# Linketic/TC-Light

Measured on AMD Instinct MI355X. Metric: relit frames/sec end-to-end (denoise+2-stage opt), higher is better.
Workload: dtype f16

## Files before the change

tc_light_amd/csrc/attn.hip:

```cpp
#include "common.h"
#include "gemm_conv.h"
#include "prof.h"
#include "../../include/tclight_hip.h"
#include <stdlib.h>
#include <type_traits>

typedef _Float16 half8 __attribute__((ext_vector_type(8)));
typedef _Float16 half4 __attribute__((ext_vector_type(4)));
typedef float float16v __attribute__((ext_vector_type(16)));
typedef float float4v __attribute__((ext_vector_type(4)));
typedef unsigned u32x4 __attribute__((ext_vector_type(4)));
typedef unsigned u32x2 __attribute__((ext_vector_type(2)));

#ifndef TCL_FLASH80_DEFAULT
#define TCL_FLASH80_DEFAULT 4
#endif
#ifndef TCL_FLASH_PV32_DEFAULT
#define TCL_FLASH_PV32_DEFAULT 0
#endif
#define KV_TILE 64
#define V_STRIDE 72
#ifndef TCL_DPV40
#define TCL_DPV40 64
#endif
// ... 36 lines not shown
        for (int j = 0; j < 8; ++j) tile[r * st + c8 + j] = x[j];
    }
    __syncthreads();
    _Float16* out = vt + ((long)bh * ntiles + tile_idx) * vt_tile_halves(DPV);
    for (int i = threadIdx.x; i < DPV * 64; i += 256) {
        int dd = i / 64, r = i % 64;
        _Float16 val = tile[r * st + dd];
        if (dd == d && DPV > d) val = (t0 + r < T) ? (_Float16)1.f : (_Float16)0.f;
        int pr = (r & ~12) | ((r & 4) << 1) | ((r & 8) >> 1);
        if (skew && (((dd & 15) + 4) & 8)) pr ^= 16;
        out[dd * V_STRIDE + pr] = val;
    }
}
__global__ __launch_bounds__(256) void k_pack_vt(const _Float16* __restrict__ v, long bstride, int ld, int T, int H, int d,
                                                 _Float16* __restrict__ vt, int ntiles, int DPV, int skew) {
    pack_vt_blk(blockIdx.x, blockIdx.y, v, bstride, ld, T, H, d, vt, ntiles, DPV, skew);
}
struct PackRows { const _Float16* src; long bstride; int ld, T, d; float scale; _Float16* dst; int Tp, DP; long total; int one_col; };
__global__ __launch_bounds__(256) void k_pack_qkv(PackRows q, PackRows k, int gq, int gk, int H, const _Float16* __restrict__ v, long vbs, int ldv, int Tk, int d,
                                                  _Float16* __restrict__ vt, int ntiles, int DPV, int skew) {
    const int blk = blockIdx.x;
    if (blk < gq) pack_rows_blk(blk, gq, q.src, q.bstride, q.ld, q.T, H, q.d, q.scale, q.dst, q.Tp, q.DP, q.total, q.one_col);
    else if (blk < gq + gk) pack_rows_blk(blk - gq, gk, k.src, k.bstride, k.ld, k.T, H, k.d, k.scale, k.dst, k.Tp, k.DP, k.total, k.one_col);
    else { const int i = blk - gq - gk; pack_vt_blk(i % ntiles, i / ntiles, v, vbs, ldv, Tk, H, d, vt, ntiles, DPV, skew); }
}

__device__ __attribute__((aligned(1024))) unsigned g_flash_zero[256];

__device__ __forceinline__ float xhalf_max(float v) {
    const auto r = __builtin_amdgcn_permlane32_swap(__float_as_uint(v), __float_as_uint(v), false, false);
    return fmaxf(__uint_as_float(r[0]), __uint_as_float(r[1]));
}

template <int D, int DP, int DPV, int QB, int NSTG, int TPB, int MINB, int SPEC, int PVW, int NW, bool SPLIT = false>
__device__ __forceinline__ void flash_block(const int bid, const _Float16* __restrict__ Qp, const _Float16* __restrict__ Kp, const _Float16* __restrict__ Vt,
                                            _Float16* __restrict__ O, int H, int Tq, int Tk, int Tqp, int Tkp, int d, int ldo, long obstride,
                                            int kv_div, int nqb, int* __restrict__ flags, float* __restrict__ lse = nullptr) {
    constexpr int KS = DP + 8;
    constexpr int NQK = DP / 16, NDT = DPV / 32;
    constexpr int KBYTES = KV_TILE * KS * 2, VBYTES = vt_tile_halves(DPV) * 2, SBYTES = KBYTES + VBYTES;
    constexpr int NPIECE = (SBYTES + 1023) / 1024, NPW = (NPIECE + NW - 1) / NW, SSTRIDE = NPIECE * 1024;
    constexpr bool LROW = DPV > D;
    constexpr bool FOLD = DP > D && LROW && (D % 16 == 8);
    constexpr bool PVQ = QB > 1;
    constexpr bool PV16 = PVW == 16 && D == 40 && LROW && DPV >= 48;
    constexpr int NT16 = 3;
    extern __shared__ __attribute__((aligned(16))) char smem[];

    const int head = bid % H, qb_ = (bid / H) % nqb, b = bid / (H * nqb);
    const int tid = threadIdx.x, lane = tid & 63, wid = __builtin_amdgcn_readfirstlane(tid >> 6), hl = lane >> 5, ql = lane & 31;
    const int q0 = qb_ * (32 * NW * QB) + wid * (32 * QB);
    const long bh = (long)b * H + head, kbh = (long)(b / kv_div) * H + head;
    const int nt = Tkp / KV_TILE, nfull = Tk / KV_TILE;
    const char* kbase = (const char*)(Kp + kbh * Tkp * KS);
    const char* vbase = (const char*)(Vt + kbh * nt * vt_tile_halves(DPV));
    const char* zero = (const char*)g_flash_zero;

#ifdef TCL_FLASH_PRIO_EXP
    if ((bid >> 3) & 1) __builtin_amdgcn_s_setprio(TCL_FLASH_PRIO_EXP);
#endif
    half8 qf[QB][NQK];
#pragma unroll
    for (int qb = 0; qb < QB; ++qb) {
        const _Float16* qrow = Qp + (bh * Tqp + q0 + qb * 32 + ql) * DP + 8 * hl;
#pragma unroll
        for (int ks = 0; ks < NQK; ++ks) qf[qb][ks] = *(const half8*)(qrow + ks * 16);
    }
    static_assert(KBYTES % 1024 == 0, "K image must be piece-aligned");
    const int lane16 = lane * 16;
    __attribute__((address_space(3))) char* const lds0 = (__attribute__((address_space(3))) char*)smem;
#define FLASH_ISSUE(IT)                                                                                                       \
    {                                                                                                                         \
        const char* kt_ = kbase + (long)(IT) * KBYTES;                                                                        \
        const char* vt_ = vbase + (long)(IT) * VBYTES;                                                                        \
        const int st_ = ((IT) % NSTG) * SSTRIDE;                                                                              \
        _Pragma("unroll") for (int i = 0; i < NPW; ++i) {                                                                    \
            const int pb_ = (wid + NW * i) * 1024;                                                                            \
            const char* src_ = (pb_ < KBYTES ? kt_ + pb_ : vt_ + (pb_ - KBYTES)) + lane16;                                    \
            if (SBYTES % 1024 != 0) src_ = pb_ + lane16 < SBYTES ? src_ : zero + lane16;                                      \
            else if (NSTG != 3 && NPW * NW != NPIECE && (wid + NW * i) >= NPIECE) continue;    \
            const int dst_ = (wid + NW * i) < NPIECE ? st_ + pb_ : NSTG * SSTRIDE;        \
            __builtin_amdgcn_global_load_lds((const __attribute__((address_space(1))) void*)src_,                             \
                                             (__attribute__((address_space(3))) void*)(lds0 + dst_), 16, 0, 0);               \
        }                                                                                                                     \
    }

    float16v o[QB][PV16 ? 1 : NDT];
    float4v o16[QB][2][PV16 ? NT16 : 1];
    float m[QB], lsum[QB];
#pragma unroll
    for (int qb = 0; qb < QB; ++qb) {
        m[qb] = FOLD ? 0.f : -1e30f; lsum[qb] = 0.f;
#pragma unroll
        for (int t = 0; t < (PV16 ? 1 : NDT); ++t)
#pragma unroll
            for (int r = 0; r < 16; ++r) o[qb][t][r] = 0.f;
#pragma unroll
        for (int qt = 0; qt < 2; ++qt)
#pragma unroll
            for (int t = 0; t < (PV16 ? NT16 : 1); ++t) o16[qb][qt][t] = float4v{0.f, 0.f, 0.f, 0.f};
    }

#ifndef TCL_SPEC_OFF
#define TCL_SPEC_OFF 3
#endif
    constexpr float OFF = TCL_SPEC_OFF;
    unsigned orv = 0;
    static_assert(!SPEC || (FOLD && (PV16 || PVQ)), "the speculative softmax is the head_dim-40 path");
    auto rebase = [&](const int it, const bool first) __attribute__((always_inline)) {
        if constexpr (SPEC) {
        const _Float16* kt = (const _Float16*)(smem + (it % NSTG) * SSTRIDE);
#pragma unroll
        for (int qb = 0; qb < QB; ++qb) {
            float16v s[2];
#pragma unroll
            for (int blk = 0; blk < 2; ++blk) {
#pragma unroll
                for (int r = 0; r < 16; ++r) s[blk][r] = 0.f;
#pragma unroll
                for (int ks = 0; ks < NQK; ++ks)
                    s[blk] = __builtin_amdgcn_mfma_f32_32x32x16_f16(*(const half8*)(kt + (blk * 32 + ql) * KS + 8 * hl + ks * 16), qf[qb][ks], s[blk], 0, 0, 0);
            }
            float mx = -1e30f;
#pragma unroll
            for (int blk = 0; blk < 2; ++blk)
#pragma unroll
                for (int r = 0; r < 16; ++r) mx = fmaxf(mx, s[blk][r]);
            mx = xhalf_max(mx) + OFF;
            const float mn = (float)(_Float16)(m[qb] + (first ? mx : fmaxf(mx, 0.f)));
            const float delta = mn - m[qb], alpha = __builtin_amdgcn_exp2f(-delta);
            m[qb] = mn;
            if (hl == 1) qf[qb][D / 16][0] = (_Float16)(-mn);
            if (!first) {
                if constexpr (PV16) {
#pragma unroll
                    for (int qt = 0; qt < 2; ++qt) {
                        const float aq = __shfl(alpha, (lane & 15) + 16 * qt, 64);
#pragma unroll
                        for (int t = 0; t < NT16; ++t) o16[qb][qt][t] *= aq;
                    }
                } else {
#pragma unroll
                    for (int t = 0; t < NDT; ++t)
#pragma unroll
                        for (int r = 0; r < 16; ++r) o[qb][t][r] *= alpha;
                }
            }
        }
        }
    };
    auto tile = [&](const int it, auto MK) __attribute__((always_inline)) {
        const _Float16* kt = (const _Float16*)(smem + (it % NSTG) * SSTRIDE);
        const _Float16* vt = kt + KV_TILE * KS;
        constexpr bool mask = decltype(MK)::value;
        half8 kf[2][NQK];
#pragma unroll
        for (int blk = 0; blk < 2; ++blk)
#pragma unroll
            for (int ks = 0; ks < NQK; ++ks) kf[blk][ks] = *(const half8*)(kt + (blk * 32 + ql) * KS + 8 * hl + ks * 16);
        half8 pf[QB][2][2];
        half8 vfr[PVQ && !PV16 ? 2 : 1][2][NDT];
        half8 vf16[PV16 ? 2 : 1][NT16];
        if constexpr (PV16) {
            const int goff = (((lane >> 4) & 1) * 16 + (lane >> 5) * 8) ^ ((((lane & 15) + 4) & 8) ? 16 : 0);
#pragma unroll
            for (int blk = 0; blk < 2; ++blk)
#pragma unroll
                for (int t = 0; t < NT16; ++t) vf16[blk][t] = *(const half8*)(vt + (t * 16 + (lane & 15)) * V_STRIDE + blk * 32 + goff);
        } else if constexpr (PVQ) {
#pragma unroll
            for (int blk = 0; blk < 2; ++blk)
#pragma unroll
                for (int ss = 0; ss < 2; ++ss)
#pragma unroll
                    for (int t = 0; t < NDT; ++t) vfr[blk][ss][t] = *(const half8*)(vt + (ql + t * 32) * V_STRIDE + blk * 32 + 16 * ss + 8 * hl);
        }
        float16v sacc[QB][2];
#pragma unroll
        for (int qb = 0; qb < QB; ++qb)
#pragma unroll
            for (int blk = 0; blk < 2; ++blk) {
#pragma unroll
                for (int r = 0; r < 16; ++r) sacc[qb][blk][r] = 0.f;
#pragma unroll
                for (int ks = 0; ks < NQK; ++ks) sacc[qb][blk] = __builtin_amdgcn_mfma_f32_32x32x16_f16(kf[blk][ks], qf[qb][ks], sacc[qb][blk], 0, 0, 0);
// ... 25 lines not shown
                        const half8 p0 = __builtin_bit_cast(half8, x), p1 = __builtin_bit_cast(half8, y);
#pragma unroll
                        for (int t = 0; t < NT16; ++t) {
                            o16[qb][0][t] = __builtin_amdgcn_mfma_f32_16x16x32_f16(vf16[blk][t], p0, o16[qb][0][t], 0, 0, 0);
                            o16[qb][1][t] = __builtin_amdgcn_mfma_f32_16x16x32_f16(vf16[blk][t], p1, o16[qb][1][t], 0, 0, 0);
                        }
                    } else {
#pragma unroll
                        for (int ss = 0; ss < 2; ++ss)
#pragma unroll
                            for (int t = 0; t < NDT; ++t) o[qb][t] = __builtin_amdgcn_mfma_f32_32x32x16_f16(vfr[blk][ss][t], pf[qb][blk][ss], o[qb][t], 0, 0, 0);
                    }
                }
            }
            if constexpr (TPB == 1) {
                if (__any((orv & 0x40004000u) != 0u)) {
                    asm volatile("; rebase");
                    rebase(it, false);
                }
                orv = 0;
            }
            return;
        }
        float mxq[QB];
#pragma unroll
        for (int qb = 0; qb < QB; ++qb) {
            float mx = sacc[qb][0][0];
#pragma unroll
            for (int blk = 0; blk < 2; ++blk)
#pragma unroll
                for (int r = 0; r < 16; ++r) mx = fmaxf(mx, sacc[qb][blk][r]);
            mxq[qb] = xhalf_max(mx);
        }
        bool need = it == 0;
#pragma unroll
        for (int qb = 0; qb < QB; ++qb) need |= FOLD ? (mxq[qb] > 6.f) : (mxq[qb] > m[qb] + 6.f);
        if (__any(need)) {
            asm volatile("; rebase");
#pragma unroll
            for (int qb = 0; qb < QB; ++qb) {
                float16v (&s)[2] = sacc[qb];
                const float mx = mxq[qb];
                if constexpr (FOLD) {
                    if (it == 0 || __any(mx > 6.f)) {
                        const float mn = (float)(_Float16)(m[qb] + (it == 0 ? mx : fmaxf(mx, 0.f)));
                        const float delta = mn - m[qb], alpha = __builtin_amdgcn_exp2f(-delta);
                        m[qb] = mn;
                        if (hl == 1) qf[qb][D / 16][0] = (_Float16)(-mn);
                        if constexpr (PV16) {
#pragma unroll
                            for (int qt = 0; qt < 2; ++qt) {
                                const float aq = __shfl(alpha, (lane & 15) + 16 * qt, 64);
#pragma unroll
                                for (int t = 0; t < NT16; ++t) o16[qb][qt][t] *= aq;
                            }
                        } else {
#pragma unroll
                            for (int t = 0; t < NDT; ++t)
#pragma unroll
                                for (int r = 0; r < 16; ++r) o[qb][t][r] *= alpha;
                        }
#pragma unroll
                        for (int blk = 0; blk < 2; ++blk)
#pragma unroll
                            for (int r = 0; r < 16; ++r) s[blk][r] -= delta;
                    }
                } else if (__any(mx > m[qb] + 6.f)) {
                    const float mn = fmaxf(m[qb], mx), alpha = __builtin_amdgcn_exp2f(m[qb] - mn);
                    m[qb] = mn;
                    lsum[qb] *= alpha;
#pragma unroll
                    for (int t = 0; t < NDT; ++t)
#pragma unroll
                        for (int r = 0; r < 16; ++r) o[qb][t][r] *= alpha;
                }
            }
        }
#pragma unroll
// ... 24 lines not shown
                    const half8 p0 = __builtin_bit_cast(half8, x), p1 = __builtin_bit_cast(half8, y);
#pragma unroll
                    for (int t = 0; t < NT16; ++t) {
                        o16[qb][0][t] = __builtin_amdgcn_mfma_f32_16x16x32_f16(vf16[blk][t], p0, o16[qb][0][t], 0, 0, 0);
                        o16[qb][1][t] = __builtin_amdgcn_mfma_f32_16x16x32_f16(vf16[blk][t], p1, o16[qb][1][t], 0, 0, 0);
                    }
                }
            } else if constexpr (PVQ) {
#pragma unroll
                for (int blk = 0; blk < 2; ++blk)
#pragma unroll
                    for (int ss = 0; ss < 2; ++ss)
#pragma unroll
                        for (int t = 0; t < NDT; ++t) o[qb][t] = __builtin_amdgcn_mfma_f32_32x32x16_f16(vfr[blk][ss][t], pf[qb][blk][ss], o[qb][t], 0, 0, 0);
            }
        }
        if constexpr (!PVQ && !PV16) {
#pragma unroll
            for (int blk = 0; blk < 2; ++blk)
#pragma unroll
                for (int ss = 0; ss < 2; ++ss) {
                    const _Float16* vr = vt + ql * V_STRIDE + blk * 32 + 16 * ss + 8 * hl;
#pragma unroll
                    for (int t = 0; t < NDT; ++t) {
                        const half8 vf = *(const half8*)(vr + t * 32 * V_STRIDE);
#pragma unroll
                        for (int qb = 0; qb < QB; ++qb) o[qb][t] = __builtin_amdgcn_mfma_f32_32x32x16_f16(vf, pf[qb][blk][ss], o[qb][t], 0, 0, 0);
                    }
                }
        }
    };
    if constexpr (TPB == 2) {
        static_assert(NSTG == 4, "two tiles per barrier need a 4-slot ring");
        FLASH_ISSUE(0);
        if (nt > 1) FLASH_ISSUE(1);
        int it = 0;
        for (; it + 1 < nfull; it += 2) {
            asm volatile("s_waitcnt vmcnt(0)" ::: "memory");
            __builtin_amdgcn_s_barrier();
            if (it + 2 < nt) FLASH_ISSUE(it + 2);
            if (it + 3 < nt) FLASH_ISSUE(it + 3);
            if (SPEC && it == 0) rebase(0, true);
            tile(it, std::false_type{});
            tile(it + 1, std::false_type{});
            if constexpr (SPEC) {
                if (__any((orv & 0x40004000u) != 0u)) {
                    asm volatile("; rebase");
                    rebase(it, false);
                    rebase(it + 1, false);
                }
                orv = 0;
            }
        }
        for (; it < nt; it += 2) {
            asm volatile("s_waitcnt vmcnt(0)" ::: "memory");
            __builtin_amdgcn_s_barrier();
            if (it + 2 < nt) FLASH_ISSUE(it + 2);
            if (it + 3 < nt) FLASH_ISSUE(it + 3);
            tile(it, std::true_type{});
            if (it + 1 < nt) tile(it + 1, std::true_type{});
        }
    } else {
        FLASH_ISSUE(0);
        if (NSTG == 3 && nt > 1) FLASH_ISSUE(1);
#define FLASH_STEP(MK)                                                                                                        \
        {                                                                                                                     \
            if (NSTG == 3 && it + 1 < nt) asm volatile("s_waitcnt vmcnt(%0)" ::"n"(NPW) : "memory");                          \
            else asm volatile("s_waitcnt vmcnt(0)" ::: "memory");                                                             \
            __builtin_amdgcn_s_barrier();              \
            if (it + NSTG - 1 < nt) FLASH_ISSUE(it + NSTG - 1);                                                               \
            if (SPEC && !decltype(MK)::value && it == 0) rebase(0, true);                                                     \
            tile(it, MK);                                                                                                     \
        }
        int it = 0;
        for (; it < nfull; ++it) FLASH_STEP(std::false_type{})
        for (; it < nt; ++it) FLASH_STEP(std::true_type{})
#undef FLASH_STEP
    }
#undef FLASH_ISSUE
    if constexpr (SPEC) {
        bool bad = false;
#pragma unroll
        for (int qb = 0; qb < QB; ++qb) {
            if constexpr (PV16) {
#pragma unroll
                for (int qt = 0; qt < 2; ++qt) { const float l = __shfl(o16[qb][qt][2][0], 32 + (lane & 15), 64); bad |= !(l > 0.f && l < 3e38f); }
            } else { const float l = o[qb][D / 32][4 * ((D % 32) / 8)]; bad |= hl == 0 && !(l > 0.f && l < 3e38f); }
        }
        const int anybad = __syncthreads_or(bad);
        if (tid == 0) flags[bid] = anybad;
    }
#pragma unroll
    for (int qb = 0; qb < QB; ++qb) {
        if constexpr (PV16) {
#pragma unroll
            for (int qt = 0; qt < 2; ++qt) {
                const float inv = 1.f / __shfl(o16[qb][qt][2][0], 32 + (lane & 15), 64);
                const int q = q0 + qb * 32 + qt * 16 + (lane & 15);
                if (q < Tq) {
                    _Float16* orow = O + (long)b * obstride + (long)q * ldo + head * d;
#pragma unroll
                    for (int t = 0; t < NT16; ++t) {
                        const int dd = t * 16 + 4 * (lane >> 4);
                        if (dd < d) {
                            const float4v v = o16[qb][qt][t];
                            half4 w = {(_Float16)(v[0] * inv), (_Float16)(v[1] * inv), (_Float16)(v[2] * inv), (_Float16)(v[3] * inv)};
                            *(half4*)(orow + dd) = w;
                        }
                    }
                }
            }
            continue;
        }
        float l;
        if (LROW) {
            constexpr int TL = D / 32, RG = (D % 32) / 8;
            l = o[qb][TL][4 * RG];
            l = __shfl(l, ql, 64);
        } else {
            l = lsum[qb] + __shfl_xor(lsum[qb], 32, 64);
        }
        const float inv = 1.f / l;
        const int q = q0 + qb * 32 + ql;
        if constexpr (SPLIT) {
            if (q < Tq && hl == 0) lse[bh * Tq + q] = m[qb] + __log2f(l);
        }
        if (q < Tq) {
            _Float16* orow = O + (long)b * obstride + (long)q * ldo + head * d;
#pragma unroll
            for (int t = 0; t < NDT; ++t)
#pragma unroll
                for (int g = 0; g < 4; ++g) {
                    int dd = t * 32 + 8 * g + 4 * hl;
                    if (dd < d) {
                        half4 w = {(_Float16)(o[qb][t][4 * g] * inv), (_Float16)(o[qb][t][4 * g + 1] * inv), (_Float16)(o[qb][t][4 * g + 2] * inv), (_Float16)(o[qb][t][4 * g + 3] * inv)};
                        *(half4*)(orow + dd) = w;
                    }
                }
        }
    }
}

template <int D, int DP, int DPV, int QB, int NSTG, int TPB, int MINB, int SPEC, int PVW, int NW>
__global__ __launch_bounds__(64 * NW, (MINB ? MINB : (QB == 1 && DP <= 80 && TPB == 1 ? 3 : 2)) * (NW >= 4 ? NW / 4 : 1)) void k_flash(const _Float16* __restrict__ Qp, const _Float16* __restrict__ Kp, const _Float16* __restrict__ Vt,
                                                  _Float16* __restrict__ O, int H, int Tq, int Tk, int Tqp, int Tkp, int d, int ldo, long obstride,
                                                  int kv_div, int nqb, int* __restrict__ flags, int nblk) {
    if constexpr (D == 40 && QB == 2 && !SPEC) {
        if (flags) {
            const int per = (nblk + (int)gridDim.x - 1) / (int)gridDim.x, lo = (int)blockIdx.x * per, hi = min(lo + per, nblk);
            for (int base = lo; base < hi; base += 64 * NW) {
                const int mine = base + (int)threadIdx.x < hi ? flags[base + threadIdx.x] : 0;
                if (!__syncthreads_or(mine)) continue;
                for (int bid = base; bid < min(base + 64 * NW, hi); ++bid) {
                    if (!flags[bid]) continue;
                    flash_block<D, DP, DPV, QB, NSTG, TPB, MINB, SPEC, PVW, NW>(bid, Qp, Kp, Vt, O, H, Tq, Tk, Tqp, Tkp, d, ldo, obstride, kv_div, nqb, flags);
                    __syncthreads();
                }
            }
            return;
        }
    }
    flash_block<D, DP, DPV, QB, NSTG, TPB, MINB, SPEC, PVW, NW>(blockIdx.x, Qp, Kp, Vt, O, H, Tq, Tk, Tqp, Tkp, d, ldo, obstride, kv_div, nqb, flags);
}

template <int NW, int NSTG>
__global__ __launch_bounds__(NW * 64, NW == 8 ? 1 : 2) void k_flash40p(const _Float16* __restrict__ Qp, const _Float16* __restrict__ Kp, const _Float16* __restrict__ Vt,
                                                    _Float16* __restrict__ O, int H, int Tq, int Tk, int Tqp, int Tkp, int ldo, long obstride,
                                                    int kv_div, int nqb) {
    constexpr int D = 40, DP = 48, DPV = 64, KS = DP + 8, NQK = 3, NT16 = 3, PF = NSTG - 3;
    constexpr int KBYTES = KV_TILE * KS * 2, VBYTES = DPV * V_STRIDE * 2, SBYTES = KBYTES + VBYTES, NPIECE = SBYTES / 1024, NPW = NPIECE / NW, SSTRIDE = SBYTES;
    static_assert(KBYTES % 1024 == 0 && NPIECE % NW == 0 && PF >= 1 && PF <= 3, "tile image must split into NW x NPW pieces");
    extern __shared__ __attribute__((aligned(16))) char smem[];
    __attribute__((address_space(3))) char* const lds0 = (__attribute__((address_space(3))) char*)smem;
    const int bid = blockIdx.x, head = bid % H, qb_ = (bid / H) % nqb, b = bid / (H * nqb);
    const int tid = threadIdx.x, lane = tid & 63, wid = __builtin_amdgcn_readfirstlane(tid >> 6), hl = lane >> 5, ql = lane & 31;
    const int q0 = qb_ * (NW * 32) + wid * 32;
    const long bh = (long)b * H + head, kbh = (long)(b / kv_div) * H + head;
    const int nt = Tkp / KV_TILE, nfull = Tk / KV_TILE;
    const char* kbase = (const char*)(Kp + kbh * Tkp * KS);
    const char* vbase = (const char*)(Vt + kbh * nt * DPV * V_STRIDE);
    const int lane16 = lane * 16, goff = (((lane >> 4) & 1) * 16 + (lane >> 5) * 8) ^ ((((lane & 15) + 4) & 8) ? 16 : 0);
    half8 qf[NQK];
    {
        const _Float16* qrow = Qp + (bh * Tqp + q0 + ql) * DP + 8 * hl;
#pragma unroll
        for (int ks = 0; ks < NQK; ++ks) qf[ks] = *(const half8*)(qrow + ks * 16);
    }
#define P40_ISSUE(IT)                                                                                                         \
    {                                                                                                                         \
        const char* kt_ = kbase + (long)(IT) * KBYTES;                                                                        \
        const char* vt_ = vbase + (long)(IT) * VBYTES;                                                                        \
        const int st_ = ((IT) % NSTG) * SSTRIDE;                                                                              \
        _Pragma("unroll") for (int i = 0; i < NPW; ++i) {                                                                    \
            const int pb_ = (wid + NW * i) * 1024;                                                                            \
            const char* src_ = (pb_ < KBYTES ? kt_ + pb_ : vt_ + (pb_ - KBYTES)) + lane16;                                    \
// ... 139 lines not shown
            _Float16* orow = O + (long)b * obstride + (long)q * ldo + head * D;
#pragma unroll
            for (int t = 0; t < NT16; ++t) {
                const int dd = t * 16 + 4 * (lane >> 4);
                if (dd < D) {
                    const float4v v = o16[qt][t];
                    half4 w = {(_Float16)(v[0] * inv), (_Float16)(v[1] * inv), (_Float16)(v[2] * inv), (_Float16)(v[3] * inv)};
                    *(half4*)(orow + dd) = w;
                }
            }
        }
    }
}

#include <vector>
#include <deque>
struct FlashProf { bool on = false; int dfilter = 0; std::deque<hipEvent_t> ev; double flops = 0.0, ms = 0.0; long launches = 0; int big[4] = {0, 0, 0, 0}; double bigfl = 0.0; };
static FlashProf g_prof;
static void flash_prof_drain(bool all) {
    while (g_prof.ev.size() >= 2) {
        hipEvent_t e0 = g_prof.ev[0], e1 = g_prof.ev[1];
        if (all) (void)hipEventSynchronize(e1);
        else if (hipEventQuery(e1) != hipSuccess) break;
        float t = 0.f;
        (void)hipEventElapsedTime(&t, e0, e1);
        g_prof.ms += t;
        (void)hipEventDestroy(e0); (void)hipEventDestroy(e1);
        g_prof.ev.pop_front(); g_prof.ev.pop_front();
    }
}

template <int D, int DP, int DPV, int QB, int NSTG, int TPB = 1, int MINB = 0, int SPEC = 0, int PVW = 16, int NW = 4>
static int launch_flash(const _Float16* Qp, const _Float16* Kp, const _Float16* Vt, _Float16* O, int B, int H, int Tq, int Tk, int Tqp, int Tkp,
                        int d, int ldo, long obs, int kv_div, hipStream_t st, int* flags = nullptr, bool count = true) {
    constexpr int SB = KV_TILE * (DP + 8) * 2 + vt_tile_halves(DPV) * 2, NPIECE = (SB + 1023) / 1024;
    const size_t lds = (size_t)NSTG * NPIECE * 1024 + 1024;
    static bool set = false;
    if (!set) { (void)hipFuncSetAttribute((const void*)k_flash<D, DP, DPV, QB, NSTG, TPB, MINB, SPEC, PVW, NW>, hipFuncAttributeMaxDynamicSharedMemorySize, (int)lds); set = true; }
    const int nqb = Tqp / (32 * NW * QB);
    const bool prof = g_prof.on && (g_prof.dfilter == 0 || g_prof.dfilter == d);
    hipEvent_t e0 = nullptr, e1 = nullptr;
    if (prof) {
        if (g_prof.ev.size() > 8192) flash_prof_drain(false);
        (void)hipEventCreate(&e0); (void)hipEventCreate(&e1); (void)hipEventRecord(e0, st);
    }
    const int nblk = B * H * nqb;
    static const int gate_blocks = getenv("TCL_FLASH_GATE_BLOCKS") ? atoi(getenv("TCL_FLASH_GATE_BLOCKS")) : 512;
    const int grid = (D == 40 && QB == 2 && !SPEC && flags && nblk > gate_blocks) ? gate_blocks : nblk;
    hipLaunchKernelGGL((k_flash<D, DP, DPV, QB, NSTG, TPB, MINB, SPEC, PVW, NW>), dim3(grid), dim3(64 * NW), lds, st, Qp, Kp, Vt, O, H, Tq, Tk, Tqp, Tkp, d, ldo, obs, kv_div, nqb, flags, nblk);
    if (prof) { (void)hipEventRecord(e1, st); g_prof.ev.push_back(e0); g_prof.ev.push_back(e1); if (count) { const double fl = 4.0 * B * H * (double)Tq * Tk * d; g_prof.flops += fl; g_prof.launches++; if (fl > g_prof.bigfl) { g_prof.bigfl = fl; g_prof.big[0] = B; g_prof.big[1] = H; g_prof.big[2] = Tq; g_prof.big[3] = Tk; } } }
    return hipPeekAtLastError() == hipSuccess ? TCL_OK : TCL_ELAUNCH;
}

template <int D, int DP, int DPV, int QB, int NSTG>
__global__ __launch_bounds__(256, 2) void k_flash_lse(const _Float16* __restrict__ Qp, const _Float16* __restrict__ Kp, const _Float16* __restrict__ Vt,
                                                      _Float16* __restrict__ O, int H, int Tq, int Tk, int Tqp, int Tkp, int d, int ldo, long obstride, int nqb,
                                                      float* __restrict__ lse) {
    flash_block<D, DP, DPV, QB, NSTG, 1, 0, 0, 16, 4, true>(blockIdx.x, Qp, Kp, Vt, O, H, Tq, Tk, Tqp, Tkp, d, ldo, obstride, 1, nqb, nullptr, lse);
}
__global__ void k_attn_merge(const _Float16* __restrict__ parts, const float* __restrict__ lse, _Float16* __restrict__ out, int S, int H, int Tq, int d, int ldo) {
    const int HD = H * d, nchunk = HD / 8;
    for (long i = (long)blockIdx.x * blockDim.x + threadIdx.x; i < (long)Tq * nchunk; i += (long)gridDim.x * blockDim.x) {
        const int q = (int)(i / nchunk), c8 = (int)(i % nchunk) * 8, h = c8 / d;
        float mx = -3.0e38f;
        for (int sidx = 0; sidx < S; ++sidx) mx = fmaxf(mx, lse[((long)sidx * H + h) * Tq + q]);
        float acc[8] = {0.f, 0.f, 0.f, 0.f, 0.f, 0.f, 0.f, 0.f}, wsum = 0.f;
        for (int sidx = 0; sidx < S; ++sidx) {
            const float wgt = exp2f(lse[((long)sidx * H + h) * Tq + q] - mx);
            const half8 pv = *(const half8*)(parts + ((long)sidx * Tq + q) * HD + c8);
            wsum += wgt;
#pragma unroll
            for (int j = 0; j < 8; ++j) acc[j] += wgt * (float)pv[j];
        }
        const float inv = 1.f / wsum;
        half8 o;
#pragma unroll
        for (int j = 0; j < 8; ++j) o[j] = (_Float16)(acc[j] * inv);
        *(half8*)(out + (long)q * ldo + c8) = o;
    }
}

static int launch_flash40p(const _Float16* Qp, const _Float16* Kp, const _Float16* Vt, _Float16* O, int B, int H, int Tq, int Tk, int Tqp, int Tkp,
                           int ldo, long obs, int kv_div, hipStream_t st) {
    constexpr int NW = 8, NSTG = 6;
    const size_t lds = (size_t)NSTG * (KV_TILE * 56 * 2 + 64 * V_STRIDE * 2);
    static bool set = false;
    if (!set) { (void)hipFuncSetAttribute((const void*)k_flash40p<NW, NSTG>, hipFuncAttributeMaxDynamicSharedMemorySize, (int)lds); set = true; }
    const int nqb = Tqp / (NW * 32);
    const bool prof = g_prof.on && (g_prof.dfilter == 0 || g_prof.dfilter == 40);
    hipEvent_t e0 = nullptr, e1 = nullptr;
    if (prof) {
        if (g_prof.ev.size() > 8192) flash_prof_drain(false);
        (void)hipEventCreate(&e0); (void)hipEventCreate(&e1); (void)hipEventRecord(e0, st);
    }
    hipLaunchKernelGGL((k_flash40p<NW, NSTG>), dim3(B * H * nqb), dim3(NW * 64), lds, st, Qp, Kp, Vt, O, H, Tq, Tk, Tqp, Tkp, ldo, obs, kv_div, nqb);
    if (prof) { (void)hipEventRecord(e1, st); g_prof.ev.push_back(e0); g_prof.ev.push_back(e1); g_prof.flops += 4.0 * B * H * (double)Tq * Tk * 40; g_prof.launches++; }
    return hipPeekAtLastError() == hipSuccess ? TCL_OK : TCL_ELAUNCH;
}

static inline int rup(int x, int m) { return (x + m - 1) / m * m; }
static int g_pv32 = -1;
static inline bool flash_pv32() {
    if (g_pv32 < 0) { const char* e = getenv("TCL_FLASH_PV"); g_pv32 = e ? (atoi(e) == 32) : TCL_FLASH_PV32_DEFAULT; }
    return g_pv32 != 0;
}

extern "C" {

int tcl_flash_profile_begin(int dfilter) { g_prof.on = true; g_prof.dfilter = dfilter; g_prof.flops = 0.0; g_prof.ms = 0.0; g_prof.launches = 0; g_prof.bigfl = 0.0; g_prof.ev.clear(); return TCL_OK; }
int tcl_flash_profile_shape(int* shape4) { TCL_CHECK_ARG(shape4); for (int i = 0; i < 4; ++i) shape4[i] = g_prof.big[i]; return TCL_OK; }
int tcl_flash_profile_end(double* total_ms, double* total_flops, long* launches) {
    TCL_CHECK_ARG(total_ms && total_flops && launches);
    flash_prof_drain(true);
    const double ms = g_prof.ms;
    *total_ms = ms; *total_flops = g_prof.flops; *launches = g_prof.launches;
    g_prof.on = false; g_prof.ev.clear();
    return TCL_OK;
}

size_t tcl_attention_q_bytes(int B, int H, int Tq, int d) { return (size_t)B * H * rup(Tq, 256) * rup(d, 16) * 2 + 256 + (size_t)B * H * (rup(Tq, 256) / 128) * 4; }
size_t tcl_attention_kv_bytes(int Bkv, int H, int Tk, int d) {
    return ((size_t)Bkv * H * rup(Tk, 64) * (rup(d, 16) + 8) + (size_t)Bkv * H * (rup(Tk, 64) / 64) * rup(d, 32) * V_STRIDE) * 2 + 2048;
}

static int attention_pack(const void* q, int ldq, long qbs, const void* k, int ldk, long kbs, const void* v, int ldv, long vbs, int B, int H, int Tq,
                          int Tk, int d, float scale, int kv_div, int pack_q, int pack_kv, void* ws_q, void* ws_kv, hipStream_t st) {
    const int Tqp = rup(Tq, 256), Tkp = rup(Tk, 64), DP = rup(d, 16), KS = DP + 8, DPV = d == 40 && !flash_pv32() ? TCL_DPV40 : rup(d, 32), Bkv = B / kv_div;
    _Float16* Qp = (_Float16*)ws_q;
    _Float16* Kp = (_Float16*)ws_kv;
    _Float16* Vt = Kp + (((size_t)Bkv * H * Tkp * KS + 511) / 512) * 512;
    long qc = (long)B * H * Tqp * (DP / 8), kc = (long)Bkv * H * Tkp * (KS / 8);
    if (pack_q && pack_kv) {
        const int gq = stream_grid(qc, 256, 2), gk = stream_grid(kc, 256, 2), nt = Tkp / 64;
        PackRows pq = {(const _Float16*)q, qbs, ldq, Tq, d, scale * 1.4426950408889634f, Qp, Tqp, DP, qc, -1};
        PackRows pk = {(const _Float16*)k, kbs, ldk, Tk, d, 1.f, Kp, Tkp, KS, kc, d == 40 ? d : -1};
        hipLaunchKernelGGL(k_pack_qkv, dim3(gq + gk + nt * Bkv * H), dim3(256), (size_t)64 * (DPV + 2) * 2, st, pq, pk, gq, gk, H, (const _Float16*)v, vbs, ldv, Tk, d, Vt,
                           nt, DPV, d == 40 && !flash_pv32() ? 1 : 0);
        return hipPeekAtLastError() == hipSuccess ? TCL_OK : TCL_ELAUNCH;
    }
    if (pack_q)
        hipLaunchKernelGGL(k_pack_rows, dim3(stream_grid(qc, 256, 2)), dim3(256), 0, st, (const _Float16*)q, qbs, ldq, Tq, H, d,
                           scale * 1.4426950408889634f, Qp, Tqp, DP, qc, -1);
    if (pack_kv) {
        hipLaunchKernelGGL(k_pack_rows, dim3(stream_grid(kc, 256, 2)), dim3(256), 0, st, (const _Float16*)k, kbs, ldk, Tk, H, d, 1.f, Kp, Tkp, KS, kc,
                           d == 40 ? d : -1);
        hipLaunchKernelGGL(k_pack_vt, dim3(Tkp / 64, Bkv * H), dim3(256), (size_t)64 * (DPV + 2) * 2, st, (const _Float16*)v, vbs, ldv, Tk, H, d, Vt, Tkp / 64, DPV, d == 40 && !flash_pv32() ? 1 : 0);
    }
    return hipPeekAtLastError() == hipSuccess ? TCL_OK : TCL_ELAUNCH;
}
int tcl_attention_pack_f16(const void* q, int ldq, long qbs, const void* k, int ldk, long kbs, const void* v, int ldv, long vbs, int B, int H, int Tq,
                           int Tk, int d, float scale, int kv_div, int pack_kv, void* ws_q, void* ws_kv, hipStream_t st) {
    TCL_CHECK_ARG(q && ws_q && ws_kv && B > 0 && H > 0 && Tq > 0 && Tk > 0 && kv_div > 0 && B % kv_div == 0);
    TCL_CHECK_ARG(d == 40 || d == 80 || d == 128 || d == 160);
// ... 13 lines not shown
}
int tcl_attention_f16(const void* q, int ldq, long qbs, const void* k, int ldk, long kbs, const void* v, int ldv, long vbs, void* o, int ldo,
                      long obs, int B, int H, int Tq, int Tk, int d, float scale, int kv_div, int pack_kv, void* ws_q, void* ws_kv,
                      hipStream_t st) {
    TCL_CHECK_ARG(q && o && ws_q && ws_kv && B > 0 && H > 0 && Tq > 0 && Tk > 0 && kv_div > 0 && B % kv_div == 0);
    TCL_CHECK_ARG(d == 40 || d == 80 || d == 128 || d == 160);
    const int pair = (pack_kv >> 1) & 1;
    const int prepacked = (pack_kv >> 2) & 1;
    pack_kv &= 1;
    TCL_CHECK_ARG(!pack_kv || (k && v));
    TCL_CHECK_ARG(!(prepacked && pack_kv));
    const int Tqp = rup(Tq, 256), Tkp = rup(Tk, 64), DP = rup(d, 16), KS = DP + 8, Bkv = B / kv_div;
    _Float16* Qp = (_Float16*)ws_q;
    _Float16* Kp = (_Float16*)ws_kv;
    _Float16* Vt = Kp + (((size_t)Bkv * H * Tkp * KS + 511) / 512) * 512;
    if (attention_pack(q, ldq, qbs, k, ldk, kbs, v, ldv, vbs, B, H, Tq, Tk, d, scale, kv_div, !prepacked, pack_kv, ws_q, ws_kv, st) != TCL_OK) return TCL_ELAUNCH;
    const bool qb2 = (long)B * (pair ? 2 : 1) * H * (Tqp / 256) >= 1024;
    static const int var40 = getenv("TCL_FLASH40") ? atoi(getenv("TCL_FLASH40")) : 0;
    if (d == 40 && var40 == 4 && TCL_DPV40 == 64 && !flash_pv32()) return launch_flash40p(Qp, Kp, Vt, (_Float16*)o, B, H, Tq, Tk, Tqp, Tkp, ldo, obs, kv_div, st);
    if (d == 40 && var40 == 2) return launch_flash<40, 48, TCL_DPV40, 1, 3>(Qp, Kp, Vt, (_Float16*)o, B, H, Tq, Tk, Tqp, Tkp, d, ldo, obs, kv_div, st);
    if (d == 40 && var40 == 3) return launch_flash<40, 48, TCL_DPV40, 1, 4, 2, 2>(Qp, Kp, Vt, (_Float16*)o, B, H, Tq, Tk, Tqp, Tkp, d, ldo, obs, kv_div, st);
    if (d == 40 && flash_pv32()) {
        if (qb2 && var40 == 0) {
            int* flags = (int*)((char*)ws_q + (((size_t)B * H * Tqp * DP * 2 + 255) / 256) * 256);
            int rc = launch_flash<40, 48, 64, 2, 4, 2, 0, 1, 32>(Qp, Kp, Vt, (_Float16*)o, B, H, Tq, Tk, Tqp, Tkp, d, ldo, obs, kv_div, st, flags);
            if (rc == TCL_OK) rc = launch_flash<40, 48, 64, 2, 4, 2, 0, 0, 32>(Qp, Kp, Vt, (_Float16*)o, B, H, Tq, Tk, Tqp, Tkp, d, ldo, obs, kv_div, st, flags, false);
            return rc;
        }
        return qb2 && var40 != 1 ? launch_flash<40, 48, 64, 2, 4, 2, 0, 0, 32>(Qp, Kp, Vt, (_Float16*)o, B, H, Tq, Tk, Tqp, Tkp, d, ldo, obs, kv_div, st)
                                 : launch_flash<40, 48, 64, 1, 2, 1, 4, 0, 32>(Qp, Kp, Vt, (_Float16*)o, B, H, Tq, Tk, Tqp, Tkp, d, ldo, obs, kv_div, st);
    }
    if (d == 40 && qb2 && var40 == 0) {
        int* flags = (int*)((char*)ws_q + (((size_t)B * H * Tqp * DP * 2 + 255) / 256) * 256);
        int rc = launch_flash<40, 48, TCL_DPV40, 2, 4, 2, 0, 1>(Qp, Kp, Vt, (_Float16*)o, B, H, Tq, Tk, Tqp, Tkp, d, ldo, obs, kv_div, st, flags);
        if (rc == TCL_OK) rc = launch_flash<40, 48, TCL_DPV40, 2, 4, 2>(Qp, Kp, Vt, (_Float16*)o, B, H, Tq, Tk, Tqp, Tkp, d, ldo, obs, kv_div, st, flags, false);
        return rc;
    }
    if (d == 40) return qb2 && var40 != 1 ? launch_flash<40, 48, TCL_DPV40, 2, 4, 2>(Qp, Kp, Vt, (_Float16*)o, B, H, Tq, Tk, Tqp, Tkp, d, ldo, obs, kv_div, st)
                                          : launch_flash<40, 48, TCL_DPV40, 1, 2, 1, 4>(Qp, Kp, Vt, (_Float16*)o, B, H, Tq, Tk, Tqp, Tkp, d, ldo, obs, kv_div, st);
    static const int var80 = getenv("TCL_FLASH80") ? atoi(getenv("TCL_FLASH80")) : TCL_FLASH80_DEFAULT;
    if (d == 80 && var80 == 8 && (long)B * H * (Tqp / 256) >= 256)
        return launch_flash<80, 80, 96, 1, 2, 1, 1, 0, 16, 8>(Qp, Kp, Vt, (_Float16*)o, B, H, Tq, Tk, Tqp, Tkp, d, ldo, obs, kv_div, st);
    if (d == 80) return launch_flash<80, 80, 96, 1, 2>(Qp, Kp, Vt, (_Float16*)o, B, H, Tq, Tk, Tqp, Tkp, d, ldo, obs, kv_div, st);
    if (d == 128) {
        static const int nw128 = getenv("TCL_FLASH128_NW") ? atoi(getenv("TCL_FLASH128_NW")) : 4;
        if (nw128 == 2)
            return launch_flash<128, 128, 128, 1, 2, 1, 0, 0, 16, 2>(Qp, Kp, Vt, (_Float16*)o, B, H, Tq, Tk, Tqp, Tkp, d, ldo, obs, kv_div, st);
        return launch_flash<128, 128, 128, 1, 2>(Qp, Kp, Vt, (_Float16*)o, B, H, Tq, Tk, Tqp, Tkp, d, ldo, obs, kv_div, st);
    }
    return launch_flash<160, 160, 160, 1, 3>(Qp, Kp, Vt, (_Float16*)o, B, H, Tq, Tk, Tqp, Tkp, d, ldo, obs, kv_div, st);
}

size_t tcl_attention_splitkv_workspace_bytes(int nsplit, int H, int Tq, int Tk, int d) {
    const size_t qb = (tcl_attention_q_bytes(nsplit, H, Tq, d) + 1023) / 1024 * 1024, kb = (tcl_attention_kv_bytes(nsplit, H, Tk / (nsplit > 0 ? nsplit : 1), d) + 1023) / 1024 * 1024;
    return qb + kb + (((size_t)nsplit * Tq * H * d * 2 + 1023) / 1024 * 1024) + (size_t)nsplit * H * Tq * 4 + 1024;
}
int tcl_attention_splitkv_f16(const void* q, int ldq, const void* k, int ldk, const void* v, int ldv, void* o, int ldo, int H, int Tq, int Tk, int d,
                              float scale, int nsplit, void* ws, hipStream_t st) {
    TCL_CHECK_ARG(q && k && v && o && ws && H > 0 && Tq > 0 && Tk > 0 && d == 128 && nsplit >= 2 && nsplit <= 16 && Tk % (64 * nsplit) == 0 && ldo >= H * d);
    const int chunk = Tk / nsplit, Tqp = rup(Tq, 256), Tkp = chunk, DP = 128, KS = DP + 8;
    char* base = (char*)ws;
    const size_t qb = (tcl_attention_q_bytes(nsplit, H, Tq, d) + 1023) / 1024 * 1024, kb = (tcl_attention_kv_bytes(nsplit, H, chunk, d) + 1023) / 1024 * 1024;
    void *ws_q = base, *ws_kv = base + qb;
    _Float16* parts = (_Float16*)(base + qb + kb);
    float* lse = (float*)(base + qb + kb + (((size_t)nsplit * Tq * H * d * 2 + 1023) / 1024 * 1024));
    if (attention_pack(q, ldq, 0, k, ldk, (long)chunk * ldk, v, ldv, (long)chunk * ldv, nsplit, H, Tq, chunk, d, scale, 1, 1, 1, ws_q, ws_kv, st) != TCL_OK) return TCL_ELAUNCH;
    _Float16* Qp = (_Float16*)ws_q;
    _Float16* Kp = (_Float16*)ws_kv;
// ... 14 lines not shown
```

Measured before the change: 5.742.

## Split KV range of tail-wave flash blocks and merge partials in the fixup kernel

```diff
diff --git a/tc_light_amd/csrc/attn.hip b/tc_light_amd/csrc/attn.hip
--- a/tc_light_amd/csrc/attn.hip
+++ b/tc_light_amd/csrc/attn.hip
@@ -92,10 +92,21 @@
     return fmaxf(__uint_as_float(r[0]), __uint_as_float(r[1]));
 }
 
+struct TailSplit {
+    int nmain, r, s, m;
+    float* part;
+    float* lse;
+    int* pflag;
+};
+
+__device__ __forceinline__ int main_bid(int x, const TailSplit& ts, int H, int nqb) { const int w = H * (nqb - ts.m), b = x / w; return b * H * nqb + (x - b * w); }
+__device__ __forceinline__ int tail_bid(int i, const TailSplit& ts, int H, int nqb) { const int w = H * ts.m, b = i / w; return b * H * nqb + (nqb - ts.m) * H + (i - b * w); }
+
 template <int D, int DP, int DPV, int QB, int NSTG, int TPB, int MINB, int SPEC, int PVW, int NW, bool SPLIT = false>
 __device__ __forceinline__ void flash_block(const int bid, const _Float16* __restrict__ Qp, const _Float16* __restrict__ Kp, const _Float16* __restrict__ Vt,
                                             _Float16* __restrict__ O, int H, int Tq, int Tk, int Tqp, int Tkp, int d, int ldo, long obstride,
-                                            int kv_div, int nqb, int* __restrict__ flags, float* __restrict__ lse = nullptr) {
+                                            int kv_div, int nqb, int* __restrict__ flags, float* __restrict__ lse = nullptr,
+                                            const int it0 = 0, int it1 = 0, float* __restrict__ part = nullptr, const int fidx = 0) {
     constexpr int KS = DP + 8;
     constexpr int NQK = DP / 16, NDT = DPV / 32;
     constexpr int KBYTES = KV_TILE * KS * 2, VBYTES = vt_tile_halves(DPV) * 2, SBYTES = KBYTES + VBYTES;
@@ -112,6 +123,7 @@
     const int q0 = qb_ * (32 * NW * QB) + wid * (32 * QB);
     const long bh = (long)b * H + head, kbh = (long)(b / kv_div) * H + head;
     const int nt = Tkp / KV_TILE, nfull = Tk / KV_TILE;
+    if (it1 == 0) it1 = nt;
     const char* kbase = (const char*)(Kp + kbh * Tkp * KS);
     const char* vbase = (const char*)(Vt + kbh * nt * vt_tile_halves(DPV));
     const char* zero = (const char*)g_flash_zero;
@@ -133,7 +145,7 @@
     {                                                                                                                         \
         const char* kt_ = kbase + (long)(IT) * KBYTES;                                                                        \
         const char* vt_ = vbase + (long)(IT) * VBYTES;                                                                        \
-        const int st_ = ((IT) % NSTG) * SSTRIDE;                                                                              \
+        const int st_ = (int)((unsigned)(IT) % NSTG) * SSTRIDE;                                                                   \
         _Pragma("unroll") for (int i = 0; i < NPW; ++i) {                                                                    \
             const int pb_ = (wid + NW * i) * 1024;                                                                            \
             const char* src_ = (pb_ < KBYTES ? kt_ + pb_ : vt_ + (pb_ - KBYTES)) + lane16;                                    \
@@ -169,7 +181,7 @@
     static_assert(!SPEC || (FOLD && (PV16 || PVQ)), "the speculative softmax is the head_dim-40 path");
     auto rebase = [&](const int it, const bool first) __attribute__((always_inline)) {
         if constexpr (SPEC) {
-        const _Float16* kt = (const _Float16*)(smem + (it % NSTG) * SSTRIDE);
+        const _Float16* kt = (const _Float16*)(smem + (unsigned)it % NSTG * SSTRIDE);
 #pragma unroll
         for (int qb = 0; qb < QB; ++qb) {
             float16v s[2];
@@ -210,7 +222,7 @@
         }
     };
     auto tile = [&](const int it, auto MK) __attribute__((always_inline)) {
-        const _Float16* kt = (const _Float16*)(smem + (it % NSTG) * SSTRIDE);
+        const _Float16* kt = (const _Float16*)(smem + (unsigned)it % NSTG * SSTRIDE);
         const _Float16* vt = kt + KV_TILE * KS;
         constexpr bool mask = decltype(MK)::value;
         half8 kf[2][NQK];
@@ -302,7 +314,7 @@
                 for (int r = 0; r < 16; ++r) mx = fmaxf(mx, sacc[qb][blk][r]);
             mxq[qb] = xhalf_max(mx);
         }
-        bool need = it == 0;
+        bool need = it == it0;
 #pragma unroll
         for (int qb = 0; qb < QB; ++qb) need |= FOLD ? (mxq[qb] > 6.f) : (mxq[qb] > m[qb] + 6.f);
         if (__any(need)) {
@@ -312,8 +324,8 @@
                 float16v (&s)[2] = sacc[qb];
                 const float mx = mxq[qb];
                 if constexpr (FOLD) {
-                    if (it == 0 || __any(mx > 6.f)) {
-                        const float mn = (float)(_Float16)(m[qb] + (it == 0 ? mx : fmaxf(mx, 0.f)));
+                    if (it == it0 || __any(mx > 6.f)) {
+                        const float mn = (float)(_Float16)(m[qb] + (it == it0 ? mx : fmaxf(mx, 0.f)));
                         const float delta = mn - m[qb], alpha = __builtin_amdgcn_exp2f(-delta);
                         m[qb] = mn;
                         if (hl == 1) qf[qb][D / 16][0] = (_Float16)(-mn);
@@ -404,15 +416,16 @@
     };
     if constexpr (TPB == 2) {
         static_assert(NSTG == 4, "two tiles per barrier need a 4-slot ring");
-        FLASH_ISSUE(0);
-        if (nt > 1) FLASH_ISSUE(1);
-        int it = 0;
-        for (; it + 1 < nfull; it += 2) {
+        FLASH_ISSUE(it0);
+        if (it0 + 1 < it1) FLASH_ISSUE(it0 + 1);
+        int it = it0;
+        const int pend = min(nfull, it1);
+        for (; it + 1 < pend; it += 2) {
             asm volatile("s_waitcnt vmcnt(0)" ::: "memory");
             __builtin_amdgcn_s_barrier();
-            if (it + 2 < nt) FLASH_ISSUE(it + 2);
-            if (it + 3 < nt) FLASH_ISSUE(it + 3);
-            if (SPEC && it == 0) rebase(0, true);
+            if (it + 2 < it1) FLASH_ISSUE(it + 2);
+            if (it + 3 < it1) FLASH_ISSUE(it + 3);
+            if (SPEC && it == it0) rebase(it0, true);
             tile(it, std::false_type{});
             tile(it + 1, std::false_type{});
             if constexpr (SPEC) {
@@ -424,13 +437,13 @@
                 orv = 0;
             }
         }
-        for (; it < nt; it += 2) {
+        for (; it < it1; it += 2) {
             asm volatile("s_waitcnt vmcnt(0)" ::: "memory");
             __builtin_amdgcn_s_barrier();
-            if (it + 2 < nt) FLASH_ISSUE(it + 2);
-            if (it + 3 < nt) FLASH_ISSUE(it + 3);
+            if (it + 2 < it1) FLASH_ISSUE(it + 2);
+            if (it + 3 < it1) FLASH_ISSUE(it + 3);
             tile(it, std::true_type{});
-            if (it + 1 < nt) tile(it + 1, std::true_type{});
+            if (it + 1 < it1) tile(it + 1, std::true_type{});
         }
     } else {
         FLASH_ISSUE(0);
@@ -460,11 +473,26 @@
             } else { const float l = o[qb][D / 32][4 * ((D % 32) / 8)]; bad |= hl == 0 && !(l > 0.f && l < 3e38f); }
         }
         const int anybad = __syncthreads_or(bad);
-        if (tid == 0) flags[bid] = anybad;
+        if (tid == 0) flags[part ? fidx : bid] = anybad;
     }
 #pragma unroll
     for (int qb = 0; qb < QB; ++qb) {
         if constexpr (PV16) {
+            if (part) {
+#pragma unroll
+                for (int qt = 0; qt < 2; ++qt) {
+                    const float l = __shfl(o16[qb][qt][2][0], 32 + (lane & 15), 64), inv = 1.f / l;
+                    const float mq = __shfl(m[qb], (lane & 15) + 16 * qt, 64);
+                    const int row = fidx * (32 * NW * QB) + wid * (32 * QB) + qb * 32 + qt * 16 + (lane & 15);
+                    if (lane < 16) lse[row] = mq + __log2f(l);
+#pragma unroll
+                    for (int t = 0; t < NT16; ++t) {
+                        const int dd = t * 16 + 4 * (lane >> 4);
+                        if (dd < D) *(float4v*)(part + (long)row * D + dd) = o16[qb][qt][t] * inv;
+                    }
+                }
+                continue;
+            }
 #pragma unroll
             for (int qt = 0; qt < 2; ++qt) {
                 const float inv = 1.f / __shfl(o16[qb][qt][2][0], 32 + (lane & 15), 64);
@@ -516,23 +544,71 @@
 template <int D, int DP, int DPV, int QB, int NSTG, int TPB, int MINB, int SPEC, int PVW, int NW>
 __global__ __launch_bounds__(64 * NW, (MINB ? MINB : (QB == 1 && DP <= 80 && TPB == 1 ? 3 : 2)) * (NW >= 4 ? NW / 4 : 1)) void k_flash(const _Float16* __restrict__ Qp, const _Float16* __restrict__ Kp, const _Float16* __restrict__ Vt,
                                                   _Float16* __restrict__ O, int H, int Tq, int Tk, int Tqp, int Tkp, int d, int ldo, long obstride,
-                                                  int kv_div, int nqb, int* __restrict__ flags, int nblk) {
+                                                  int kv_div, int nqb, int* __restrict__ flags, int nblk, const TailSplit ts) {
     if constexpr (D == 40 && QB == 2 && !SPEC) {
         if (flags) {
-            const int per = (nblk + (int)gridDim.x - 1) / (int)gridDim.x, lo = (int)blockIdx.x * per, hi = min(lo + per, nblk);
+            const int nscan = ts.r ? ts.nmain : nblk;
+            const int per = (nscan + (int)gridDim.x - 1) / (int)gridDim.x, lo = (int)blockIdx.x * per, hi = min(lo + per, nscan);
             for (int base = lo; base < hi; base += 64 * NW) {
-                const int mine = base + (int)threadIdx.x < hi ? flags[base + threadIdx.x] : 0;
+                const int mine = base + (int)threadIdx.x < hi ? flags[ts.r ? main_bid(base + threadIdx.x, ts, H, nqb) : base + threadIdx.x] : 0;
                 if (!__syncthreads_or(mine)) continue;
-                for (int bid = base; bid < min(base + 64 * NW, hi); ++bid) {
+                for (int x = base; x < min(base + 64 * NW, hi); ++x) {
+                    const int bid = ts.r ? main_bid(x, ts, H, nqb) : x;
                     if (!flags[bid]) continue;
                     flash_block<D, DP, DPV, QB, NSTG, TPB, MINB, SPEC, PVW, NW>(bid, Qp, Kp, Vt, O, H, Tq, Tk, Tqp, Tkp, d, ldo, obstride, kv_div, nqb, flags);
                     __syncthreads();
                 }
             }
+            static_assert(32 * NW * QB == 256 && D % 4 == 0, "one row per thread of a 256-query item");
+            for (int i = (int)blockIdx.x; i < ts.r; i += (int)gridDim.x) {
+                const int bid = tail_bid(i, ts, H, nqb);
+                const int bad = __syncthreads_or((int)threadIdx.x < ts.s ? ts.pflag[threadIdx.x * ts.r + i] : 0);
+                if (threadIdx.x == 0) flags[bid] = bad;
+                if (bad) {
+                    flash_block<D, DP, DPV, QB, NSTG, TPB, MINB, SPEC, PVW, NW>(bid, Qp, Kp, Vt, O, H, Tq, Tk, Tqp, Tkp, d, ldo, obstride, kv_div, nqb, flags);
+                    __syncthreads();
+                    continue;
+                }
+                const int head = bid % H, b = bid / (H * nqb), q = ((bid / H) % nqb) * 256 + (int)threadIdx.x;
+                if (q >= Tq) continue;
+                float mx = -3.0e38f;
+                for (int k = 0; k < ts.s; ++k) mx = fmaxf(mx, ts.lse[(k * ts.r + i) * 256 + threadIdx.x]);
+                float4v acc[D / 4];
+#pragma unroll
+                for (int c = 0; c < D / 4; ++c) acc[c] = float4v{0.f, 0.f, 0.f, 0.f};
+                float wsum = 0.f;
+                for (int k = 0; k < ts.s; ++k) {
+                    const long row = (long)(k * ts.r + i) * 256 + threadIdx.x;
+                    const float w = __builtin_amdgcn_exp2f(ts.lse[row] - mx);
+                    wsum += w;
+#pragma unroll
+                    for (int c = 0; c < D / 4; ++c) acc[c] += w * *(const float4v*)(ts.part + row * D + 4 * c);
+                }
+                const float inv = 1.f / wsum;
+                _Float16* orow = O + (long)b * obstride + (long)q * ldo + head * d;
+#pragma unroll
+                for (int c = 0; c < D / 4; ++c) {
+                    const float4v v = acc[c] * inv;
+                    *(half4*)(orow + 4 * c) = half4{(_Float16)v[0], (_Float16)v[1], (_Float16)v[2], (_Float16)v[3]};
+                }
+            }
             return;
         }
     }
-    flash_block<D, DP, DPV, QB, NSTG, TPB, MINB, SPEC, PVW, NW>(blockIdx.x, Qp, Kp, Vt, O, H, Tq, Tk, Tqp, Tkp, d, ldo, obstride, kv_div, nqb, flags);
+    int bid = blockIdx.x, it0 = 0, it1 = 0, fidx = 0;
+    int* fl = flags;
+    float *part = nullptr, *plse = nullptr;
+    if constexpr (SPEC && PVW == 16) {
+        if (ts.r && bid >= ts.nmain) {
+            const int j = bid - ts.nmain, i = j % ts.r, k = j / ts.r, np = Tkp / (2 * KV_TILE);
+            it0 = 2 * ((k * np) / ts.s);
+            it1 = k + 1 == ts.s ? Tkp / KV_TILE : 2 * (((k + 1) * np) / ts.s);
+            bid = tail_bid(i, ts, H, nqb); fidx = j; fl = ts.pflag; part = ts.part; plse = ts.lse;
+        } else if (ts.r) {
+            bid = main_bid(bid, ts, H, nqb);
+        }
+    }
+    flash_block<D, DP, DPV, QB, NSTG, TPB, MINB, SPEC, PVW, NW>(bid, Qp, Kp, Vt, O, H, Tq, Tk, Tqp, Tkp, d, ldo, obstride, kv_div, nqb, fl, plse, it0, it1, part, fidx);
 }
 
 template <int NW, int NSTG>
@@ -738,7 +814,7 @@
 
 template <int D, int DP, int DPV, int QB, int NSTG, int TPB = 1, int MINB = 0, int SPEC = 0, int PVW = 16, int NW = 4>
 static int launch_flash(const _Float16* Qp, const _Float16* Kp, const _Float16* Vt, _Float16* O, int B, int H, int Tq, int Tk, int Tqp, int Tkp,
-                        int d, int ldo, long obs, int kv_div, hipStream_t st, int* flags = nullptr, bool count = true) {
+                        int d, int ldo, long obs, int kv_div, hipStream_t st, int* flags = nullptr, bool count = true, const TailSplit ts = TailSplit{}) {
     constexpr int SB = KV_TILE * (DP + 8) * 2 + vt_tile_halves(DPV) * 2, NPIECE = (SB + 1023) / 1024;
     const size_t lds = (size_t)NSTG * NPIECE * 1024 + 1024;
     static bool set = false;
@@ -752,8 +828,8 @@
     }
     const int nblk = B * H * nqb;
     static const int gate_blocks = getenv("TCL_FLASH_GATE_BLOCKS") ? atoi(getenv("TCL_FLASH_GATE_BLOCKS")) : 512;
-    const int grid = (D == 40 && QB == 2 && !SPEC && flags && nblk > gate_blocks) ? gate_blocks : nblk;
-    hipLaunchKernelGGL((k_flash<D, DP, DPV, QB, NSTG, TPB, MINB, SPEC, PVW, NW>), dim3(grid), dim3(64 * NW), lds, st, Qp, Kp, Vt, O, H, Tq, Tk, Tqp, Tkp, d, ldo, obs, kv_div, nqb, flags, nblk);
+    const int grid = (D == 40 && QB == 2 && !SPEC && flags && nblk > gate_blocks) ? gate_blocks : SPEC && ts.r ? ts.nmain + ts.r * ts.s : nblk;
+    hipLaunchKernelGGL((k_flash<D, DP, DPV, QB, NSTG, TPB, MINB, SPEC, PVW, NW>), dim3(grid), dim3(64 * NW), lds, st, Qp, Kp, Vt, O, H, Tq, Tk, Tqp, Tkp, d, ldo, obs, kv_div, nqb, flags, nblk, ts);
     if (prof) { (void)hipEventRecord(e1, st); g_prof.ev.push_back(e0); g_prof.ev.push_back(e1); if (count) { const double fl = 4.0 * B * H * (double)Tq * Tk * d; g_prof.flops += fl; g_prof.launches++; if (fl > g_prof.bigfl) { g_prof.bigfl = fl; g_prof.big[0] = B; g_prof.big[1] = H; g_prof.big[2] = Tq; g_prof.big[3] = Tk; } } }
     return hipPeekAtLastError() == hipSuccess ? TCL_OK : TCL_ELAUNCH;
 }
@@ -811,6 +887,36 @@
     return g_pv32 != 0;
 }
 
+static int resident_slots() {
+    static int slots[64] = {0};
+    int dev = 0;
+    (void)hipGetDevice(&dev);
+    if (dev < 0 || dev >= 64) dev = 0;
+    if (!slots[dev]) {
+        int cus = 0;
+        if (hipDeviceGetAttribute(&cus, hipDeviceAttributeMultiprocessorCount, dev) != hipSuccess || cus <= 0) cus = 256;
+        slots[dev] = 2 * cus;
+    }
+    return slots[dev];
+}
+static size_t tail_ws_offset(int B, int H, int Tq) {
+    return ((size_t)B * H * rup(Tq, 256) * 48 * 2 + 255) / 256 * 256 + ((size_t)B * H * (rup(Tq, 256) / 128) * 4 + 255) / 256 * 256;
+}
+static size_t tail_ws_bytes() { return (size_t)resident_slots() * (256 * 41 * 4 + 4); }
+static TailSplit tail_split(int B, int H, int Tq, int Tkp, void* ws_q, int pair) {
+    static const int on = getenv("TCL_FLASH_TAILSPLIT") ? atoi(getenv("TCL_FLASH_TAILSPLIT")) : 1;
+    TailSplit ts{};
+    const int R = resident_slots(), nqb = rup(Tq, 256) / 256, bh = B * (pair ? 2 : 1) * H, rem = (bh * nqb) % R, m = (rem + bh - 1) / bh;
+    const int s = rem && m < nqb ? min(min(8, R / (bh * m)), Tkp / (2 * KV_TILE)) : 0;
+    if (!on || s < 2) return ts;
+    char* base = (char*)ws_q + tail_ws_offset(B, H, Tq);
+    ts.r = B * H * m; ts.nmain = B * H * nqb - ts.r; ts.s = s; ts.m = m;
+    ts.part = (float*)base;
+    ts.lse = (float*)(base + (size_t)R * 256 * 40 * 4);
+    ts.pflag = (int*)(base + (size_t)R * 256 * 41 * 4);
+    return ts;
+}
+
 extern "C" {
 
 int tcl_flash_profile_begin(int dfilter) { g_prof.on = true; g_prof.dfilter = dfilter; g_prof.flops = 0.0; g_prof.ms = 0.0; g_prof.launches = 0; g_prof.bigfl = 0.0; g_prof.ev.clear(); return TCL_OK; }
@@ -824,7 +930,9 @@
     return TCL_OK;
 }
 
-size_t tcl_attention_q_bytes(int B, int H, int Tq, int d) { return (size_t)B * H * rup(Tq, 256) * rup(d, 16) * 2 + 256 + (size_t)B * H * (rup(Tq, 256) / 128) * 4; }
+size_t tcl_attention_q_bytes(int B, int H, int Tq, int d) {
+    return d == 40 ? tail_ws_offset(B, H, Tq) + tail_ws_bytes() + 256 : (size_t)B * H * rup(Tq, 256) * rup(d, 16) * 2 + 256 + (size_t)B * H * (rup(Tq, 256) / 128) * 4;
+}
 size_t tcl_attention_kv_bytes(int Bkv, int H, int Tk, int d) {
     return ((size_t)Bkv * H * rup(Tk, 64) * (rup(d, 16) + 8) + (size_t)Bkv * H * (rup(Tk, 64) / 64) * rup(d, 32) * V_STRIDE) * 2 + 2048;
 }
@@ -904,8 +1012,9 @@
     }
     if (d == 40 && qb2 && var40 == 0) {
         int* flags = (int*)((char*)ws_q + (((size_t)B * H * Tqp * DP * 2 + 255) / 256) * 256);
-        int rc = launch_flash<40, 48, TCL_DPV40, 2, 4, 2, 0, 1>(Qp, Kp, Vt, (_Float16*)o, B, H, Tq, Tk, Tqp, Tkp, d, ldo, obs, kv_div, st, flags);
-        if (rc == TCL_OK) rc = launch_flash<40, 48, TCL_DPV40, 2, 4, 2>(Qp, Kp, Vt, (_Float16*)o, B, H, Tq, Tk, Tqp, Tkp, d, ldo, obs, kv_div, st, flags, false);
+        const TailSplit ts = tail_split(B, H, Tq, Tkp, ws_q, pair);
+        int rc = launch_flash<40, 48, TCL_DPV40, 2, 4, 2, 0, 1>(Qp, Kp, Vt, (_Float16*)o, B, H, Tq, Tk, Tqp, Tkp, d, ldo, obs, kv_div, st, flags, true, ts);
+        if (rc == TCL_OK) rc = launch_flash<40, 48, TCL_DPV40, 2, 4, 2>(Qp, Kp, Vt, (_Float16*)o, B, H, Tq, Tk, Tqp, Tkp, d, ldo, obs, kv_div, st, flags, false, ts);
         return rc;
     }
     if (d == 40) return qb2 && var40 != 1 ? launch_flash<40, 48, TCL_DPV40, 2, 4, 2>(Qp, Kp, Vt, (_Float16*)o, B, H, Tq, Tk, Tqp, Tkp, d, ldo, obs, kv_div, st)
```

New measurement: 5.727, median of 2. No clear change (-0.3%).
